# zama-ai/bounty-matrix-inversion

Measured on AMD Instinct MI355X. Metric: PBS/sec per GPU + encrypted n x n inverse wall-clock (n=2,3,4), higher is better.
Workload: dtype u64/f64

## Files before the change

bounty-matrix-inversion_amd/csrc/bmi_host.cpp:

```cpp
#include <hip/hip_runtime.h>

#include <errno.h>
#include <sys/random.h>

#include <algorithm>
#include <cmath>
#include <cstdio>
#include <cstring>
#include <string>
#include <thread>
#include <vector>

#include "../../include/bmi_tfhe.h"
#include "bmi_internal.hpp"
#include "field49.hpp"
#include "ntt_wave.hpp"
#include "ntt_half_f64.hpp"
#include "ntt_wave_f64.hpp"
#include "fft_half_f64.hpp"
#include "fft_wave_f64.hpp"
#include "fft_eighth_f64.hpp"
#include "fft_quarter_f64.hpp"
#include "t64_common.hpp"

// ... 615 lines not shown
    const int prec = c->bsk_prec;
    const hipStream_t st = c->stream;
    const char *what = "bsk_to_lat (unrolled key)";
    int rc;
    if (c->t64() && bmit::shape_supported_unrolled_fft(prec, c->P.bs_levels, c->P.bs_base_log))
        rc = build_copy(c, c->bsk3.fft_lat, bytes, what,
                        [&](double *d) { return bmit::launch_bsk_to_latf(std_polys, d, c->tw_fft_half.get(), polys, prec, st); });
    else if (c->t64())
        rc = build_copy(c, c->bsk3.exact_lat, bytes, what,
                        [&](double *d) { return bmit::launch_bsk_to_lat(std_polys, d, c->tw_half.get(), polys, prec, st); });
    else if (c->wide())
        rc = build_copy(c, c->bsk3.wide49, bytes, what,
                        [&](double *d) { return bmi49::launch_bsk_to_wide(std_polys, d, c->tw_wave.get(), c->tw_wide49.get(), polys, st); });
    else
        rc = build_copy(c, c->bsk3.lat49, bytes, what,
                        [&](double *d) { return bmi49::launch_bsk_to_lat(std_polys, d, c->tw_half.get(), polys, true, st); });
    if (rc) return rc;
    c->have_bsk3 = true;
    return 0;
}

const FieldOps GOLDILOCKS_OPS = {bmi::launch_keyswitch, bmi::launch_keyswitch_mfma, bmi::launch_ksk_to_limbs, bmi::launch_lincomb, bmi::launch_lwe_phase,
    [](bmi_ctx *c, const u64 *std_polys) { return build_copy(c, c->bsk.ntt_gl, c->bsk_std.size() * 8, "bsk_to_ntt", [&](u64 *d) {
        return bmi::launch_bsk_to_ntt(std_polys, d, c->tw_gl.get(), (uint32_t)(c->bsk_std.size() / c->N), c->stream); }); },
    [](const bmi_ctx *c, const u64 *a, const u64 *b, u64 *o, uint32_t m) { return bmi::launch_negacyclic_mul(a, b, o, c->tw_gl.get(), m, c->stream); },
    bmi::KS_LIMBS};
const FieldOps FIELD49_OPS = {bmi49::launch_keyswitch, bmi49::launch_keyswitch_mfma, bmi49::launch_ksk_to_limbs, bmi49::launch_lincomb, bmi49::launch_lwe_phase,
    [](bmi_ctx *c, const u64 *std_polys) { return build_copy(c, c->bsk.ntt49, c->bsk_std.size() * 8, "bsk_to_ntt", [&](double *d) {
        return bmi49::launch_bsk_to_ntt(std_polys, d, c->tw_wave.get(), (uint32_t)(c->bsk_std.size() / c->N), c->stream); }); },
    [](const bmi_ctx *c, const u64 *a, const u64 *b, u64 *o, uint32_t m) { return bmi49::launch_negacyclic_mul(a, b, o, c->tw_wave.get(), m, c->stream); },
    bmi49::KS_LIMBS};
const FieldOps TORUS64_OPS = {bmit::launch_keyswitch, bmit::launch_keyswitch_mfma, bmit::launch_ksk_to_limbs, bmit::launch_lincomb, bmit::launch_lwe_phase,
                              nullptr, nullptr, bmit::KS_LIMBS};

int gen_eval_keys(bmi_ctx *c, uint64_t seed) {
    HIP_OK(c, hipSetDevice(c->device));
    drop_sk_mask(c);
    const bmi_params &P = c->P;
    const uint32_t n = P.n, N = c->N, k = P.k, lk = P.ks_levels, rows = c->rows;
    c->seed = seed;
    if (!c->secure_rng) c->enc_counter = 0;
    c->bsk_std.assign((size_t)n * rows * (k + 1) * N, 0);
    gen_ggsw_rows(c, seed, S_BSK_MASK, S_BSK_NOISE, c->sk_small, c->bsk_std.data());
    c->have_bsk3 = false;
    if (c->unroll == 2) gen_bsk3(c, seed);
    c->ksk.assign((size_t)k * N * lk * (n + 1), 0);
    {
        const Stream sm_det(seed, S_KSK_MASK, c->f), se_det(seed, S_KSK_NOISE, c->f);
        const Stream *smp = &sm_det, *sep = &se_det;
        const ChaKey *ksec = &c->rng_secret, *kpub = &c->rng_public;
        const bool secure = c->secure_rng;
        const Fq f = c->f;
        const u64 *skb = c->sk_big.data();
        const u64 *sks = c->sk_small.data();
        u64 *ksk = c->ksk.data();
        const double sigma = P.lwe_noise;
        const uint32_t bl = P.ks_base_log;
        parallel_for((size_t)k * N * lk, [=](size_t jr) {
            RowRng sm(smp, *kpub, S_KSK_MASK, jr, secure), se(sep, *ksec, S_KSK_NOISE, jr, secure);
            const uint32_t j = (uint32_t)(jr / lk), lev = (uint32_t)(jr % lk);
            u64 *row = ksk + jr * (n + 1);
            u64 b = se.gauss(jr, sigma);
            for (uint32_t x = 0; x < n; x++) {
                row[x] = sm.uniform((u64)jr * (n + 1) + x);
                if (sks[x]) b = f.add(b, row[x]);
            }
            if (skb[j]) b = f.add(b, (u64)1 << (f.bits - bl * (lev + 1)));
            row[n] = b;
        });
    }
    c->have_secret = true;
    if (int rc = upload_eval_keys(c)) return rc;
    return c->unroll == 2 ? upload_bsk3(c) : 0;
}

uint32_t ks_mfma_slices(const bmi_ctx *c, uint32_t count) {
    const uint32_t tiles = (count + 31) / 32, cbs = (c->P.n + 1 + 31) / 32;
    const uint32_t ksteps = c->big_n * c->P.ks_levels / 32;
    uint32_t slices = 1;
    while (slices < 64 && slices * 2 <= ksteps && ksteps % (slices * 2) == 0 && (size_t)tiles * cbs * slices < 2048) slices *= 2;
    return slices;
}

int ensure_ks_mfma(bmi_ctx *c, uint32_t count) {
    const uint32_t cbs = (c->P.n + 1 + 31) / 32;
    const size_t sums = (size_t)ks_mfma_slices(c, count) * count * c->ops->ks_limbs * cbs * 32 * sizeof(int);
    const int rc = grow(c, c->ks_digits, (size_t)count * c->big_n * c->P.ks_levels, (size_t)8 << 20);
    return rc ? rc : grow(c, c->ks_sums, sums, (size_t)32 << 20);
}

enum class Rot {
    t64_wide2, t64_wide, t64_quad, t64_tp2u_fft, t64_lat2u_fft, t64_lat2u, t64_lat_fft, t64_lat, t64_fft, t64_exact,
    f49_wide_u, f49_wide, f49_quad, f49_lat2u, f49_lat2, f49_tpx,
    gl_lat, gl_tp,
};

int choose_rotation(const bmi_ctx *c, uint32_t count, Rot *rot) {
    if (c->unroll == 2 && !c->have_bsk3)
        return fail(c, -1, "unrolling selected but the context holds no unrolled key: generate keys after bmi_set_bsk_unroll, or bmi_import_bsk_unrolled");
    const int v = c->variant;
    const bool latency = v == 2 || (v == 0 && count <= c->lat_threshold);
    const bool two_per_wg = v == 1 || v == 3 || (v == 0 && count > 256);
    const int prec = c->bsk_prec;
    const uint32_t lv = c->P.bs_levels, bl = c->P.bs_base_log;
    if (c->t64()) {
        if (c->wide() && !c->bsk.wide2.empty() && two_per_wg) *rot = Rot::t64_wide2;
        else if (c->wide()) *rot = Rot::t64_wide;
        else if (c->quad()) *rot = Rot::t64_quad;
        else if (c->unroll == 2)
            *rot = !bmit::shape_supported_unrolled_fft(prec, lv, bl) ? Rot::t64_lat2u : two_per_wg ? Rot::t64_tp2u_fft : Rot::t64_lat2u_fft;
        else {
            if (c->bsk.fft.empty() && !bmit::shape_supported(prec, lv, bl))
                return fail(c, -1, "this bootstrap-key precision exists for the unrolled kernel only: bmi_set_bsk_unroll(ctx, 2) before keygen");
            if ((v == 5 || v == 6) && c->bsk.fft.empty())
                return fail(c, -1, "kernel variant " + std::to_string(v) + " needs the bootstrap key at 48 bits of precision in base 2^10 (the torus default)");
            const bool lat_t = v == 2 || v == 4 || v == 6 || (v == 0 && count <= c->lat_threshold);
            const bool fft = !c->bsk.fft.empty() && (lat_t ? v != 4 : v == 0 || v == 5);
            *rot = lat_t ? (fft ? Rot::t64_lat_fft : Rot::t64_lat) : (fft ? Rot::t64_fft : Rot::t64_exact);
        }
    } else if (c->f64()) {
        if (c->wide()) *rot = c->unroll == 2 ? Rot::f49_wide_u : Rot::f49_wide;
        else if (c->quad()) *rot = Rot::f49_quad;
        else *rot = c->unroll == 2 ? Rot::f49_lat2u : latency ? Rot::f49_lat2 : Rot::f49_tpx;
    } else {
        *rot = latency ? Rot::gl_lat : Rot::gl_tp;
    }
    return 0;
}

int launch_rotation(const bmi_ctx *c, Rot rot, const u64 *cts, const uint32_t *ids, uint32_t count, u64 *out, unsigned long long *stat,
                    hipStream_t st) {
    const uint32_t n = c->P.n, lv = c->P.bs_levels, bl = c->P.bs_base_log;
    const int p = c->bsk_prec;
    const u64 *luts = c->luts.get();
    const double *luts49 = reinterpret_cast<const double *>(luts);
    const bmi_ctx::BskCopies &K = c->bsk;
    const bmi_ctx::Bsk3Copies &K3 = c->bsk3;
    switch (rot) {
    case Rot::t64_wide2: return bmit::launch_blind_rotate_wide2(cts, ids, luts, K.wide2.get(), c->tw_quarter.get(), out, count, n, p, lv, bl, st);
    case Rot::t64_wide: return bmit::launch_blind_rotate_wide(cts, ids, luts, K.wide.get(), c->tw_quarter.get(), out, count, n, p, lv, bl, stat, st);
    case Rot::t64_quad: return bmit::launch_blind_rotate_quad(cts, ids, luts, K.quad.get(), c->tw_eighth.get(), out, count, n, p, lv, bl, stat, st);
    case Rot::t64_tp2u_fft: return bmit::launch_blind_rotate_tp2u_fft(cts, ids, luts, K3.fft_lat.get(), c->tw_fft_half.get(), c->zeta_pow.get(), out,
                                                                      count, n, p, lv, bl, st);
    case Rot::t64_lat2u_fft: return bmit::launch_blind_rotate_lat2u_fft(cts, ids, luts, K3.fft_lat.get(), c->tw_fft_half.get(), c->zeta_pow.get(),
                                                                        out, count, n, p, lv, bl, stat, st);
    case Rot::t64_lat2u: return bmit::launch_blind_rotate_lat2u(cts, ids, luts, K3.exact_lat.get(), c->tw_half.get(), c->root_pow.get(), out, count,
                                                                n, p, lv, bl, st);
    case Rot::t64_lat_fft: return bmit::launch_blind_rotate_lat_fft(cts, ids, luts, K.fft_lat.get(), c->tw_fft_half.get(), out, count, n, p, lv, bl, stat, st);
    case Rot::t64_lat: return bmit::launch_blind_rotate_lat(cts, ids, luts, K.exact_lat.get(), c->tw_half.get(), out, count, n, p, lv, bl, st);
    case Rot::t64_fft: return bmit::launch_blind_rotate_fft(cts, ids, luts, K.fft.get(), c->tw_fft.get(), out, count, n, p, lv, bl, stat, st);
    case Rot::t64_exact: return bmit::launch_blind_rotate(cts, ids, luts, K.exact.get(), c->tw_wave.get(), out, count, n, p, lv, bl, st);
    case Rot::f49_wide_u: return bmi49::launch_blind_rotate_wide_u(cts, ids, luts49, K3.wide49.get(), c->tw_wave.get(), c->tw_wide49.get(),
                                                                   c->root_pow.get(), out, count, n, lv, bl, st);
    case Rot::f49_wide: return bmi49::launch_blind_rotate_wide(cts, ids, luts49, K.wide49.get(), c->tw_wave.get(), c->tw_wide49.get(), out, count, n, lv, bl, st);
    case Rot::f49_quad: return bmi49::launch_blind_rotate_quad(cts, ids, luts49, K.quad49.get(), c->tw_wave.get(), c->tw_quad49.get(), out, count, n, st);
    case Rot::f49_lat2u: return bmi49::launch_blind_rotate_lat2u(cts, ids, luts49, K3.lat49.get(), c->tw_half.get(), c->root_pow.get(), out, count, n, lv, bl, st);
    case Rot::f49_lat2: return bmi49::launch_blind_rotate_lat2(cts, ids, luts49, K.lat49.get(), c->tw_half.get(), out, count, n, lv, bl, st);
    case Rot::f49_tpx: return bmi49::launch_blind_rotate_tpx(cts, ids, luts49, K.ntt49.get(), c->tw_wave.get(), out, count, n, lv, bl, st);
    case Rot::gl_lat: return bmi::launch_blind_rotate_lat(cts, ids, luts, K.ntt_gl.get(), c->tw_gl.get(), out, count, n, st);
    case Rot::gl_tp: return bmi::launch_blind_rotate_tp(cts, ids, luts, K.ntt_gl.get(), c->tw_gl.get(), out, count, n, st);
    }
    return (int)hipErrorInvalidValue;
}

int check_lut_ids(bmi_ctx *c, const uint32_t *lut_ids, uint32_t count) {
    for (uint32_t i = 0; i < count; i++)
        if (lut_ids[i] >= c->n_luts) return fail(c, -1, "look-up id " + std::to_string(lut_ids[i]) + " is not registered");
    return 0;
}

}
// ... 440 lines not shown
        while (slices < 64 && tiles * slices * 2 <= 1024) slices *= 2;
    if (slices > 1)
        if (int rc = grow(c, c->ks_partial, (size_t)slices * count * c->ks_stride * 16, KS_PARTIAL_BYTES)) return rc;
    int rc = c->ops->keyswitch(d_in, c->ksk_padded.get(), c->ks_bias.get(), d_small, slices > 1 ? c->ks_partial.get() : nullptr, slices,
                               count, c->P.n, c->big_n, c->P.ks_levels, c->P.ks_base_log, c->ks_stride, (hipStream_t)stream);
    return rc ? fail(c, -2, std::string("keyswitch launch: ") + hipGetErrorString((hipError_t)rc)) : 0;
}

int bmi_blind_rotate_batch(bmi_ctx *c, const uint64_t *d_small, const uint32_t *d_lut_ids, uint32_t count,
                           uint64_t *d_out, void *stream) {
    if (!c || (count && (!d_small || !d_lut_ids || !d_out))) return -1;
    if (!c->have_keys) return fail(c, -1, "no keys: call bmi_keygen first");
    HIP_OK(c, hipSetDevice(c->device));
    Rot rot;
    if (int rc = choose_rotation(c, count, &rot)) return rc;
    if (rot == Rot::t64_lat || rot == Rot::t64_exact)
        if (int rc = build_exact_torus_copies(c, nullptr)) return rc;
    const int rc = launch_rotation(c, rot, d_small, d_lut_ids, count, d_out, nullptr, (hipStream_t)stream);
    return rc ? fail(c, -2, std::string("blind_rotate launch: ") + hipGetErrorString((hipError_t)rc)) : 0;
}

int bmi_pbs_batch(bmi_ctx *c, const uint64_t *d_in, const uint32_t *d_lut_ids, uint32_t count, uint64_t *d_out,
                  void *stream) {
    if (!c) return -1;
    HIP_OK(c, hipSetDevice(c->device));
    int rc = ensure_small(c, count);
    if (rc) return rc;
    rc = bmi_keyswitch_batch(c, d_in, count, c->small.get(), stream);
    if (rc) return rc;
    return bmi_blind_rotate_batch(c, c->small.get(), d_lut_ids, count, d_out, stream);
}

int bmi_lincomb_batch(bmi_ctx *c, const uint64_t *d_store, const uint32_t *d_row_ptr, const uint32_t *d_idx,
                      const int64_t *d_coef, const uint64_t *d_const_body, uint32_t count, uint64_t *d_out,
                      void *stream) {
    if (!c || (count && (!d_store || !d_row_ptr || !d_const_body || !d_out))) return -1;
    HIP_OK(c, hipSetDevice(c->device));
    int rc = c->ops->lincomb(d_store, d_row_ptr, d_idx, (const i64 *)d_coef, d_const_body, d_out, count, c->big_n + 1, (hipStream_t)stream);
    return rc ? fail(c, -2, std::string("lincomb launch: ") + hipGetErrorString((hipError_t)rc)) : 0;
}

static int phase_decrypt_batch(bmi_ctx *c, const uint64_t *d_ct, uint32_t count, uint32_t delta_log, const int64_t *d_expected,
                               uint64_t *d_phase, int64_t *d_msgs, int64_t *d_err, void *stream) {
    if (!c->have_keys) return fail(c, -1, "no keys: call bmi_keygen first");
    if (!c->have_secret) return fail(c, -1, "evaluation-only context: it holds no secret key");
    if (count == 0) return 0;
    HIP_OK(c, hipSetDevice(c->device));
    if (int rc = ensure_sk_mask(c)) return rc;
    const int rc = c->ops->lwe_phase(d_ct, c->sk_mask.get(), d_phase, (const i64 *)d_expected, (i64 *)d_msgs, (i64 *)d_err, count, c->big_n,
                                     delta_log, (hipStream_t)stream);
    return rc ? fail(c, -2, std::string("lwe_phase launch: ") + hipGetErrorString((hipError_t)rc)) : 0;
}

int bmi_phase_batch(bmi_ctx *c, const uint64_t *d_ct, uint32_t count, uint64_t *d_phase, void *stream) {
    if (!c || (count && (!d_ct || !d_phase))) return -1;
    return phase_decrypt_batch(c, d_ct, count, 0, nullptr, d_phase, nullptr, nullptr, stream);
}

int bmi_decrypt_batch(bmi_ctx *c, const uint64_t *d_ct, uint32_t count, uint32_t delta_log, const int64_t *d_expected,
                      int64_t *d_msgs, int64_t *d_err, void *stream) {
    if (!c || (count && (!d_ct || !d_msgs))) return -1;
    if (delta_log == 0 || delta_log >= c->f.bits - 1) return fail(c, -1, "delta_log out of range");
    return phase_decrypt_batch(c, d_ct, count, delta_log, d_expected, nullptr, d_msgs, d_err, stream);
}

int bmi_scatter_rows(bmi_ctx *c, const uint64_t *d_src, uint32_t count, uint64_t *d_store, const uint32_t *d_rows,
                     void *stream) {
    if (!c || (count && (!d_src || !d_store || !d_rows))) return -1;
    HIP_OK(c, hipSetDevice(c->device));
    int rc = bmi::launch_scatter_rows(d_src, d_store, d_rows, count, c->big_n + 1, (hipStream_t)stream);
    return rc ? fail(c, -2, std::string("scatter_rows launch: ") + hipGetErrorString((hipError_t)rc)) : 0;
}

int bmi_reserve(bmi_ctx *c, uint32_t max_count) {
    if (!c) return -1;
    HIP_OK(c, hipSetDevice(c->device));
    HIP_OK(c, hipDeviceSynchronize());
    if (int rc = grow(c, c->ks_partial, KS_PARTIAL_BYTES, KS_PARTIAL_BYTES)) return rc;
    if (c->ks_mfma_ok) {
        uint32_t worst = max_count;
        size_t worst_sums = 0;
        for (uint32_t tiles = 1; tiles <= (max_count + 31) / 32; tiles++) {
            const uint32_t cnt = std::min(tiles * 32, max_count);
            const size_t sums = (size_t)ks_mfma_slices(c, cnt) * cnt;
            if (sums > worst_sums) { worst_sums = sums; worst = cnt; }
        }
        int rc = ensure_ks_mfma(c, worst);
        if (rc) return rc;
        rc = ensure_ks_mfma(c, max_count);
        if (rc) return rc;
    }
    return ensure_small(c, max_count);
}

int bmi_sync(bmi_ctx *c, void *stream) {
    if (!c) return -1;
    HIP_OK(c, hipStreamSynchronize((hipStream_t)stream));
    return 0;
}

int bmi_pbs_batch_host(bmi_ctx *c, const uint64_t *in, const uint32_t *lut_ids, uint32_t count, uint64_t *out) {
    if (!c || !in || !lut_ids || !out) return -1;
    if (int bad = check_lut_ids(c, lut_ids, count)) return bad;
    HIP_OK(c, hipSetDevice(c->device));
    int rc = ensure_io(c, count);
    if (rc) return rc;
    const size_t w = (size_t)(c->big_n + 1) * 8;
    HIP_OK(c, hipMemcpyAsync(c->io_a.get(), in, count * w, hipMemcpyHostToDevice, c->stream));
    HIP_OK(c, hipMemcpyAsync(c->io_ids.get(), lut_ids, count * 4, hipMemcpyHostToDevice, c->stream));
    rc = bmi_pbs_batch(c, c->io_a.get(), c->io_ids.get(), count, c->io_b.get(), c->stream);
    if (rc) return rc;
    HIP_OK(c, hipMemcpyAsync(out, c->io_b.get(), count * w, hipMemcpyDeviceToHost, c->stream));
    HIP_OK(c, hipStreamSynchronize(c->stream));
    return 0;
}

int bmi_keyswitch_batch_host(bmi_ctx *c, const uint64_t *in, uint32_t count, uint64_t *small_out) {
    if (!c || !in || !small_out) return -1;
    HIP_OK(c, hipSetDevice(c->device));
    int rc = ensure_io(c, count);
    if (rc) return rc;
    HIP_OK(c, hipMemcpyAsync(c->io_a.get(), in, (size_t)count * (c->big_n + 1) * 8, hipMemcpyHostToDevice, c->stream));
    rc = bmi_keyswitch_batch(c, c->io_a.get(), count, c->small.get(), c->stream);
    if (rc) return rc;
    HIP_OK(c, hipMemcpyAsync(small_out, c->small.get(), (size_t)count * (c->P.n + 1) * 8, hipMemcpyDeviceToHost, c->stream));
    HIP_OK(c, hipStreamSynchronize(c->stream));
    return 0;
}

int bmi_blind_rotate_batch_host(bmi_ctx *c, const uint64_t *small_in, const uint32_t *lut_ids, uint32_t count,
                                uint64_t *out) {
    if (!c || !small_in || !lut_ids || !out) return -1;
    if (int bad = check_lut_ids(c, lut_ids, count)) return bad;
    HIP_OK(c, hipSetDevice(c->device));
    int rc = ensure_io(c, count);
    if (rc) return rc;
    HIP_OK(c, hipMemcpyAsync(c->small.get(), small_in, (size_t)count * (c->P.n + 1) * 8, hipMemcpyHostToDevice, c->stream));
    HIP_OK(c, hipMemcpyAsync(c->io_ids.get(), lut_ids, count * 4, hipMemcpyHostToDevice, c->stream));
    rc = bmi_blind_rotate_batch(c, c->small.get(), c->io_ids.get(), count, c->io_b.get(), c->stream);
    if (rc) return rc;
    HIP_OK(c, hipMemcpyAsync(out, c->io_b.get(), (size_t)count * (c->big_n + 1) * 8, hipMemcpyDeviceToHost, c->stream));
    HIP_OK(c, hipStreamSynchronize(c->stream));
    return 0;
}

int bmi_fft_margin_host(bmi_ctx *c, const uint64_t *small_in, const uint32_t *lut_ids, uint32_t count, uint64_t *out,
                        double *max_distance) {
    if (!c || !small_in || !lut_ids || !out || !max_distance) return -1;
    if (!c->have_keys) return fail(c, -1, "no keys: call bmi_keygen first");
    const bool ufft = c->t64() && c->unroll == 2 && c->have_bsk3 && bmit::shape_supported_unrolled_fft(c->bsk_prec, c->P.bs_levels, c->P.bs_base_log);
    const bool wide_key = !c->bsk.wide.empty() || !c->bsk.quad.empty();
    if (c->bsk.fft.empty() && !wide_key && !ufft)
        return fail(c, -1, "the floating-point-transform kernels exist on the 2^64 torus with the bootstrap key at 48 bits (N = 1024), 46 bits "
                           "(N = 2048) or 44 bits (N = 4096) in base 2^10");
    const Rot rot = ufft ? Rot::t64_lat2u_fft : !wide_key && (c->variant == 6 || c->variant == 2) ? Rot::t64_lat_fft
                    : wide_key ? (c->quad() ? Rot::t64_quad : Rot::t64_wide) : Rot::t64_fft;
    if (int bad = check_lut_ids(c, lut_ids, count)) return bad;
    HIP_OK(c, hipSetDevice(c->device));
    int rc = ensure_io(c, count);
    if (rc) return rc;
    DevBuf<unsigned long long> d_stat;
    HIP_OK(c, d_stat.alloc(8));
    hipError_t e = hipMemsetAsync(d_stat.get(), 0, 8, c->stream);
    if (e == hipSuccess) e = hipMemcpyAsync(c->small.get(), small_in, (size_t)count * (c->P.n + 1) * 8, hipMemcpyHostToDevice, c->stream);
    if (e == hipSuccess) e = hipMemcpyAsync(c->io_ids.get(), lut_ids, count * 4, hipMemcpyHostToDevice, c->stream);
    if (e == hipSuccess) e = (hipError_t)launch_rotation(c, rot, c->small.get(), c->io_ids.get(), count, c->io_b.get(), d_stat.get(), c->stream);
    unsigned long long bits = 0;
// ... 26 lines not shown
```

bounty-matrix-inversion_amd/csrc/bmi_internal.hpp:

```cpp
#pragma once
#include <hip/hip_runtime.h>
#include <stdint.h>

#include "goldilocks.hpp"

#ifndef BMI_DEFAULT_Q_BITS
#define BMI_DEFAULT_Q_BITS 65
#endif

#ifndef BMI_TPX49_PF
#define BMI_TPX49_PF 13
#endif

#ifndef BMI_TPX49_RESYNC
#define BMI_TPX49_RESYNC 4
#endif

#define BMI_LUT_CAP 1024
#define BMI_MAX_LWE_N 1024
constexpr int BMI_AT_WORDS = 264;
constexpr int BMI_LDS_WORDS_MAX = 160 * 1024 / 8;
#ifndef BMI_KS_MFMA_MIN
#define BMI_KS_MFMA_MIN 1
#endif
// ... 33 lines not shown
    BMI_LAUNCH_CHECK();
    return 0;
}

template <typename F>
inline int with_levels(uint32_t levels, F f) {
    if (levels == 3) return f(std::integral_constant<int, 3>{});
    return f(std::integral_constant<int, 2>{});
}
template <typename F>
inline int with_levels_stats(uint32_t levels, bool stats, F f) {
    return with_levels(levels, [&](auto L) { return stats ? f(L, std::true_type{}) : f(L, std::false_type{}); });
}

namespace bmi {
using gl::i64;
using gl::u64;

int launch_bsk_to_ntt(const u64 *std_polys, u64 *ntt_polys, const u64 *g_tw, uint32_t n_polys, hipStream_t s);
int launch_negacyclic_mul(const u64 *a, const u64 *b, u64 *c, const u64 *g_tw, uint32_t count, hipStream_t s);
int launch_blind_rotate_tp(const u64 *small_cts, const uint32_t *lut_ids, const u64 *luts, const u64 *bsk,
                           const u64 *g_tw, u64 *out, uint32_t count, uint32_t n, hipStream_t s);
int launch_blind_rotate_lat(const u64 *small_cts, const uint32_t *lut_ids, const u64 *luts, const u64 *bsk,
                            const u64 *g_tw, u64 *out, uint32_t count, uint32_t n, hipStream_t s);
int launch_keyswitch(const u64 *in, const u64 *ksk, const u64 *ks_bias, u64 *out, void *partial, uint32_t slices,
                     uint32_t count, uint32_t n, uint32_t big_n, uint32_t levels, uint32_t base_log, uint32_t ks_stride,
                     hipStream_t s);
constexpr uint32_t KS_LIMBS = 9;
int launch_ksk_to_limbs(const u64 *ksk, signed char *limbs, uint32_t rows, uint32_t n, uint32_t ks_stride, hipStream_t s);
int launch_keyswitch_mfma(const u64 *in, const signed char *limbs, signed char *digits, int *sums, u64 *out,
                          uint32_t slices, uint32_t count, uint32_t n, uint32_t big_n, uint32_t levels,
                          uint32_t base_log, hipStream_t s);
int launch_lincomb(const u64 *store, const uint32_t *row_ptr, const uint32_t *idx, const i64 *coef,
                   const u64 *const_body, u64 *out, uint32_t count, uint32_t width, hipStream_t s);
int launch_scatter_rows(const u64 *src, u64 *store, const uint32_t *rows, uint32_t count, uint32_t width, hipStream_t s);
int launch_lwe_phase(const u64 *ct, const u64 *key_mask, u64 *phase, const i64 *expected, i64 *msgs, i64 *err,
                     uint32_t count, uint32_t big_n, uint32_t delta_log, hipStream_t s);
}

namespace bmi49 {
using gl::i64;
using gl::u64;
int launch_bsk_to_ntt(const u64 *std_polys, double *ntt_polys, const double *g_tw, uint32_t n_polys, hipStream_t s);
int launch_negacyclic_mul(const u64 *a, const u64 *b, u64 *c, const double *g_tw, uint32_t count, hipStream_t s);
int launch_bsk_to_quad(const u64 *std_polys, double *quad_polys, const double *g_tw, const double *g_t, uint32_t n_polys,
                       hipStream_t s);
int launch_blind_rotate_quad(const u64 *small_cts, const uint32_t *lut_ids, const double *luts, const double *bsk_quad,
                             const double *g_tw, const double *g_t, u64 *out, uint32_t count, uint32_t n, hipStream_t s);
int launch_bsk_to_wide(const u64 *std_polys, double *wide_polys, const double *g_tw, const double *g_tw_wide,
                       uint32_t n_polys, hipStream_t s);
int launch_blind_rotate_wide(const u64 *small_cts, const uint32_t *lut_ids, const double *luts, const double *bsk_wide,
                             const double *g_tw, const double *g_tw_wide, u64 *out, uint32_t count, uint32_t n,
                             uint32_t levels, uint32_t base_log, hipStream_t s);
int launch_blind_rotate_wide_u(const u64 *small_cts, const uint32_t *lut_ids, const double *luts, const double *bsk3_wide,
                               const double *g_tw, const double *g_tw_wide, const double *g_root_pow, u64 *out, uint32_t count,
                               uint32_t n, uint32_t levels, uint32_t base_log, hipStream_t s);
int launch_bsk_to_lat(const u64 *std_polys, double *lat_polys, const double *g_tw_h, uint32_t n_polys, bool paired, hipStream_t s);
int launch_blind_rotate_lat2(const u64 *small_cts, const uint32_t *lut_ids, const double *luts, const double *bsk_lat,
                             const double *g_tw_h, u64 *out, uint32_t count, uint32_t n, uint32_t levels, uint32_t base_log,
                             hipStream_t s);
int launch_blind_rotate_lat2u(const u64 *small_cts, const uint32_t *lut_ids, const double *luts, const double *bsk3_lat,
                              const double *g_tw_h, const double *g_root_pow, u64 *out, uint32_t count, uint32_t n,
                              uint32_t levels, uint32_t base_log, hipStream_t s);
int launch_blind_rotate_tpx(const u64 *small_cts, const uint32_t *lut_ids, const double *luts, const double *bsk,
                            const double *g_tw, u64 *out, uint32_t count, uint32_t n, uint32_t levels, uint32_t base_log,
                            hipStream_t s);
int launch_keyswitch(const u64 *in, const u64 *ksk, const u64 *ks_bias, u64 *out, void *partial, uint32_t slices,
                     uint32_t count, uint32_t n, uint32_t big_n, uint32_t levels, uint32_t base_log, uint32_t ks_stride,
                     hipStream_t s);
constexpr uint32_t KS_LIMBS = 7;
int launch_ksk_to_limbs(const u64 *ksk, signed char *limbs, uint32_t rows, uint32_t n, uint32_t ks_stride, hipStream_t s);
int launch_keyswitch_mfma(const u64 *in, const signed char *limbs, signed char *digits, int *sums, u64 *out,
                          uint32_t slices, uint32_t count, uint32_t n, uint32_t big_n, uint32_t levels,
                          uint32_t base_log, hipStream_t s);
int launch_lincomb(const u64 *store, const uint32_t *row_ptr, const uint32_t *idx, const i64 *coef,
                   const u64 *const_body, u64 *out, uint32_t count, uint32_t width, hipStream_t s);
int launch_lwe_phase(const u64 *ct, const u64 *key_mask, u64 *phase, const i64 *expected, i64 *msgs, i64 *err,
                     uint32_t count, uint32_t big_n, uint32_t delta_log, hipStream_t s);
}

namespace bmit {
using gl::i64;
using gl::u64;
constexpr uint32_t KS_LIMBS = 9;
bool shape_supported(int prec, uint32_t levels, uint32_t base_log);
bool shape_supported_unrolled(int prec, uint32_t levels, uint32_t base_log);
int launch_bsk_to_limbs(const u64 *std_polys, double *limb_polys, const double *g_tw, uint32_t n_polys, int prec,
                        hipStream_t s);
int launch_blind_rotate(const u64 *small_cts, const uint32_t *lut_ids, const u64 *luts, const double *bsk_limbs,
                        const double *g_tw, u64 *out, uint32_t count, uint32_t n, int prec, uint32_t levels,
                        uint32_t base_log, hipStream_t s);
int launch_bsk_to_lat(const u64 *std_polys, double *lat_polys, const double *g_tw_h, uint32_t n_polys, int prec, hipStream_t s);
int launch_blind_rotate_lat(const u64 *small_cts, const uint32_t *lut_ids, const u64 *luts, const double *bsk_lat,
                            const double *g_tw_h, u64 *out, uint32_t count, uint32_t n, int prec, uint32_t levels,
                            uint32_t base_log, hipStream_t s);
int launch_blind_rotate_lat2u(const u64 *small_cts, const uint32_t *lut_ids, const u64 *luts, const double *bsk3_lat,
                              const double *g_tw_h, const double *g_root_pow, u64 *out, uint32_t count, uint32_t n, int prec,
                              uint32_t levels, uint32_t base_log, hipStream_t s);
bool shape_supported_fft(int prec, uint32_t levels, uint32_t base_log);
int launch_bsk_to_fft(const u64 *std_polys, double *limb_polys, const double *g_tw_fft, uint32_t n_polys, int prec, hipStream_t s);
int launch_blind_rotate_fft(const u64 *small_cts, const uint32_t *lut_ids, const u64 *luts, const double *bsk_fft,
                            const double *g_tw_fft, u64 *out, uint32_t count, uint32_t n, int prec, uint32_t levels,
                            uint32_t base_log, unsigned long long *stat, hipStream_t s);
int launch_bsk_to_latf(const u64 *std_polys, double *lat_polys, const double *g_tw_h, uint32_t n_polys, int prec, hipStream_t s);
int launch_blind_rotate_lat_fft(const u64 *small_cts, const uint32_t *lut_ids, const u64 *luts, const double *bsk_fft,
                                const double *g_tw_fft, u64 *out, uint32_t count, uint32_t n, int prec, uint32_t levels,
                                uint32_t base_log, unsigned long long *stat, hipStream_t s);
bool shape_supported_unrolled_fft(int prec, uint32_t levels, uint32_t base_log);
int launch_blind_rotate_lat2u_fft(const u64 *small_cts, const uint32_t *lut_ids, const u64 *luts, const double *bsk3_latf,
                                  const double *g_tw_h, const double *g_zeta_pow, u64 *out, uint32_t count, uint32_t n, int prec,
                                  uint32_t levels, uint32_t base_log, unsigned long long *stat, hipStream_t s);
int launch_blind_rotate_tp2u_fft(const u64 *small_cts, const uint32_t *lut_ids, const u64 *luts, const double *bsk3_latf,
                                 const double *g_tw_h, const double *g_zeta_pow, u64 *out, uint32_t count, uint32_t n, int prec,
                                 uint32_t levels, uint32_t base_log, hipStream_t s);
bool shape_supported_quad(int prec, uint32_t levels, uint32_t base_log);
int launch_bsk_to_quad(const u64 *std_polys, double *q_polys, const double *g_tw_e, uint32_t n_polys, int prec, hipStream_t s);
int launch_blind_rotate_quad(const u64 *small_cts, const uint32_t *lut_ids, const u64 *luts, const double *bsk_q, const double *g_tw_e,
                             u64 *out, uint32_t count, uint32_t n, int prec, uint32_t levels, uint32_t base_log, unsigned long long *stat,
                             hipStream_t s);
int launch_bsk_to_wide2(const u64 *std_polys, double *w2_polys, const double *g_tw_q, uint32_t n_polys, int prec, hipStream_t s);
int launch_blind_rotate_wide2(const u64 *small_cts, const uint32_t *lut_ids, const u64 *luts, const double *bsk_w2, const double *g_tw_q,
                              u64 *out, uint32_t count, uint32_t n, int prec, uint32_t levels, uint32_t base_log, hipStream_t s);
bool shape_supported_wide(int prec, uint32_t levels, uint32_t base_log);
int launch_bsk_to_wide(const u64 *std_polys, double *w_polys, const double *g_tw_q, uint32_t n_polys, int prec, hipStream_t s);
int launch_blind_rotate_wide(const u64 *small_cts, const uint32_t *lut_ids, const u64 *luts, const double *bsk_w, const double *g_tw_q,
                             u64 *out, uint32_t count, uint32_t n, int prec, uint32_t levels, uint32_t base_log, unsigned long long *stat,
                             hipStream_t s);
int launch_keyswitch(const u64 *in, const u64 *ksk, const u64 *ks_bias, u64 *out, void *partial, uint32_t slices,
                     uint32_t count, uint32_t n, uint32_t big_n, uint32_t levels, uint32_t base_log, uint32_t ks_stride,
                     hipStream_t s);
int launch_ksk_to_limbs(const u64 *ksk, signed char *limbs, uint32_t rows, uint32_t n, uint32_t ks_stride, hipStream_t s);
int launch_keyswitch_mfma(const u64 *in, const signed char *limbs, signed char *digits, int *sums, u64 *out,
                          uint32_t slices, uint32_t count, uint32_t n, uint32_t big_n, uint32_t levels,
                          uint32_t base_log, hipStream_t s);
int launch_lincomb(const u64 *store, const uint32_t *row_ptr, const uint32_t *idx, const i64 *coef,
                   const u64 *const_body, u64 *out, uint32_t count, uint32_t width, hipStream_t s);
int launch_lwe_phase(const u64 *ct, const u64 *key_mask, u64 *phase, const i64 *expected, i64 *msgs, i64 *err,
                     uint32_t count, uint32_t big_n, uint32_t delta_log, hipStream_t s);
}
```

bounty-matrix-inversion_amd/csrc/ks_mfma.hpp:

```cpp
#pragma once
#include <hip/hip_runtime.h>
#include <stdint.h>

#include "bmi_internal.hpp"

namespace ksm {

typedef uint64_t u64;
typedef int64_t i64;
typedef int v4i __attribute__((ext_vector_type(4)));
typedef int v16i __attribute__((ext_vector_type(16)));

constexpr int TILE = 32;
constexpr int KSTEP = 32;
constexpr int WAVES = 4;
#ifndef BMI_KS_PF_WIDE
#define BMI_KS_PF_WIDE 3
#endif
#ifndef BMI_KS_PF
#define BMI_KS_PF 4
#endif

template <class F>
__global__ void __launch_bounds__(256)
    k_ks_digits(const u64 *__restrict__ in, signed char *__restrict__ D, uint32_t count, uint32_t big_n, uint32_t levels,
                uint32_t base_log) {
    const size_t idx = (size_t)blockIdx.x * blockDim.x + threadIdx.x;
    if (idx >= (size_t)count * big_n) return;
    const uint32_t ct = (uint32_t)(idx / big_n), j = (uint32_t)(idx % big_n);
    unsigned char d[16];
    F::digits(in[(size_t)ct * (big_n + 1) + j], levels, base_log, d);
    const int half = 1 << (base_log - 1);
    signed char *o = D + ((size_t)ct * big_n + j) * levels;
    if ((levels & 7) == 0) {
        for (uint32_t g = 0; g < levels; g += 8) {
            u64 w = 0;
#pragma unroll
            for (int lev = 0; lev < 8; lev++) w |= (u64)(unsigned char)(signed char)((int)d[g + lev] - half) << (8 * lev);
            *reinterpret_cast<u64 *>(o + g) = w;
        }
    } else {
        for (uint32_t lev = 0; lev < levels; lev++) o[lev] = (signed char)((int)d[lev] - half);
    }
}

__host__ __device__ __forceinline__ size_t limb_offset(uint32_t cb, uint32_t ks, uint32_t limb, uint32_t h, uint32_t r,
                                                       uint32_t ksteps, uint32_t L) {
    return (((((size_t)cb * ksteps + ks) * L + limb) * 2 + h) * 32 + r) * 16;
}

template <class F>
__global__ void __launch_bounds__(256)
    k_ksk_to_limbs(const u64 *__restrict__ ksk, signed char *__restrict__ Bm, uint32_t rows, uint32_t n, uint32_t ks_stride,
                   uint32_t L) {
    const uint32_t cbs = (n + 1 + TILE - 1) / TILE, ksteps = rows / KSTEP;
    const size_t idx = (size_t)blockIdx.x * blockDim.x + threadIdx.x;
    if (idx >= (size_t)rows * cbs * TILE) return;
    const uint32_t col = (uint32_t)(idx % (cbs * TILE)), k = (uint32_t)(idx / (cbs * TILE));
    __int128 c = col <= n ? (__int128)F::centered(ksk[(size_t)k * ks_stride + col]) : 0;
    const uint32_t cb = col / TILE, r = col % TILE, ks = k / KSTEP, h = (k % KSTEP) / 16, byte = k % 16;
    for (uint32_t l = 0; l < L; l++) {
        const int dl = (int)((c + 128) & 255) - 128;
        c = (c - dl) >> 8;
        Bm[limb_offset(cb, ks, l, h, r, ksteps, L) + byte] = (signed char)dl;
    }
}

template <int L>
constexpr int ks_pf() { return L <= 7 ? BMI_KS_PF : BMI_KS_PF_WIDE; }

template <int L>
__global__ void __launch_bounds__(64 * WAVES)
    k_ks_mfma(const signed char *__restrict__ D, const signed char *__restrict__ Bm, int *__restrict__ S, uint32_t count,
              uint32_t K, uint32_t cbs, uint32_t ksteps_per_slice) {
    const int wave = threadIdx.x >> 6, lane = threadIdx.x & 63;
    const uint32_t tile = blockIdx.x * WAVES + wave;
    if (tile * TILE >= count) return;
    const uint32_t cb = blockIdx.y, slice = blockIdx.z;
    const uint32_t r = lane & 31, h = lane >> 5;
    const uint32_t ksteps = K / KSTEP;
    const uint32_t ks0 = slice * ksteps_per_slice;
    const uint32_t ks1 = min(ks0 + ksteps_per_slice, ksteps);
    const uint32_t ct_row = min(tile * TILE + r, count - 1);
    const v4i *ap = reinterpret_cast<const v4i *>(D + (size_t)ct_row * K + 16 * h) + (size_t)ks0 * 2;
    const v4i *bp = reinterpret_cast<const v4i *>(Bm + limb_offset(cb, ks0, 0, h, r, ksteps, L));
    constexpr int BSTEP = L * 64;

    v16i acc[L];
#pragma unroll
    for (int l = 0; l < L; l++)
#pragma unroll
        for (int i = 0; i < 16; i++) acc[l][i] = 0;

    constexpr int KS_PF = ks_pf<L>();
    v4i a_buf[KS_PF], b_buf[KS_PF][L];
#pragma unroll
    for (int s = 0; s < KS_PF; s++) {
        a_buf[s] = v4i{0, 0, 0, 0};
#pragma unroll
        for (int l = 0; l < L; l++) b_buf[s][l] = v4i{0, 0, 0, 0};
        if (ks0 + s < ks1) {
            a_buf[s] = ap[2 * s];
#pragma unroll
            for (int l = 0; l < L; l++) b_buf[s][l] = bp[s * BSTEP + l * 64];
        }
    }
    for (uint32_t ks = ks0; ks < ks1; ks += KS_PF) {
#pragma unroll
        for (int s = 0; s < KS_PF; s++) {
            if (ks + s < ks1) {
#pragma unroll
                for (int l = 0; l < L; l++) acc[l] = __builtin_amdgcn_mfma_i32_32x32x32_i8(a_buf[s], b_buf[s][l], acc[l], 0, 0, 0);
                if (ks + s + KS_PF < ks1) {
                    a_buf[s] = ap[2 * (s + KS_PF)];
#pragma unroll
                    for (int l = 0; l < L; l++) b_buf[s][l] = bp[(s + KS_PF) * BSTEP + l * 64];
                }
            }
        }
        ap += 2 * KS_PF;
        bp += (size_t)BSTEP * KS_PF;
    }

    const uint32_t cw = cbs * TILE;
#pragma unroll
    for (int i = 0; i < 16; i++) {
        const uint32_t row = (i & 3) + 8 * (i >> 2) + 4 * h;
        const uint32_t ct = tile * TILE + row;
        if (ct >= count) continue;
        int *o = S + (((size_t)slice * count + ct) * L) * cw + cb * TILE + r;
#pragma unroll
        for (int l = 0; l < L; l++) o[(size_t)l * cw] = acc[l][i];
    }
}

template <class F, int L>
__global__ void __launch_bounds__(256)
    k_ks_combine(const u64 *__restrict__ in, const int *__restrict__ S, u64 *__restrict__ out, uint32_t count, uint32_t n,
                 uint32_t big_n, uint32_t cbs, uint32_t slices) {
    const uint32_t ct = blockIdx.x;
    const uint32_t cw = cbs * TILE;
    for (uint32_t col = threadIdx.x; col <= n; col += blockDim.x) {
        i64 sum[L];
#pragma unroll
        for (int l = 0; l < L; l++) sum[l] = 0;
#pragma unroll 4
        for (uint32_t sl = 0; sl < slices; sl++) {
            const int *base = S + (((size_t)sl * count + ct) * L) * cw + col;
#pragma unroll
            for (int l = 0; l < L; l++) sum[l] += base[(size_t)l * cw];
        }
        __int128 v = 0;
#pragma unroll
        for (int l = L - 1; l >= 0; l--) v = v * 256 + sum[l];
        const bool neg = v < 0;
        const unsigned __int128 m = neg ? (unsigned __int128)(-v) : (unsigned __int128)v;
        u64 red = F::reduce128((u64)(m >> 64), (u64)m);
        if (neg) red = F::neg(red);
        const u64 base = col == n ? in[(size_t)ct * (big_n + 1) + big_n] : 0;
        out[(size_t)ct * (n + 1) + col] = F::sub(base, red);
    }
}

inline size_t limb_bytes(uint32_t rows, uint32_t n, uint32_t L) {
    const uint32_t cbs = (n + 1 + TILE - 1) / TILE;
    return (size_t)cbs * (rows / KSTEP) * L * 2 * 32 * 16;
}
inline size_t s_bytes(uint32_t count, uint32_t n, uint32_t L, uint32_t slices) {
    const uint32_t cbs = (n + 1 + TILE - 1) / TILE;
    return (size_t)slices * count * L * cbs * TILE * sizeof(int);
}

template <class F>
int launch_ksk_to_limbs(const u64 *ksk, signed char *Bm, uint32_t rows, uint32_t n, uint32_t ks_stride, uint32_t L,
                        hipStream_t s) {
    const uint32_t cbs = (n + 1 + TILE - 1) / TILE;
    const size_t total = (size_t)rows * cbs * TILE;
    hipLaunchKernelGGL((k_ksk_to_limbs<F>), dim3((unsigned)((total + 255) / 256)), dim3(256), 0, s, ksk, Bm, rows, n,
                       ks_stride, L);
    BMI_LAUNCH_CHECK();
    return 0;
}

template <class F, int L>
int launch_keyswitch(const u64 *in, const signed char *Bm, signed char *D, int *S, u64 *out, uint32_t slices,
                     uint32_t count, uint32_t n, uint32_t big_n, uint32_t levels, uint32_t base_log, hipStream_t s) {
    if (count == 0) return 0;
    const uint32_t K = big_n * levels, cbs = (n + 1 + TILE - 1) / TILE, ksteps = K / KSTEP;
    const size_t coefs = (size_t)count * big_n;
    hipLaunchKernelGGL((k_ks_digits<F>), dim3((unsigned)((coefs + 255) / 256)), dim3(256), 0, s, in, D, count, big_n, levels,
                       base_log);
    BMI_LAUNCH_CHECK();
    const uint32_t tiles = (count + TILE - 1) / TILE;
    const uint32_t per_slice = (ksteps + slices - 1) / slices;
    hipLaunchKernelGGL((k_ks_mfma<L>), dim3((tiles + WAVES - 1) / WAVES, cbs, slices), dim3(64 * WAVES), 0, s, D, Bm, S, count,
                       K, cbs, per_slice);
    BMI_LAUNCH_CHECK();
    hipLaunchKernelGGL((k_ks_combine<F, L>), dim3(count), dim3(256), 0, s, in, S, out, count, n, big_n, cbs, slices);
    BMI_LAUNCH_CHECK();
    return 0;
}

}
```

Measured before the change: 121,100.

## Stage keyswitch MFMA B-tiles through LDS and fuse combine when unsliced

The int8 MFMA keyswitch kernel now loads the key-limb tiles cooperatively into a double-buffered shared-memory stage, with register prefetch, instead of each wave loading its own copy from global memory. When only one K-slice is used, recombination and reduction are fused into the MFMA epilogue, which skips the partial-sum buffer and the separate combine launch. The T64 keyswitch limb count drops from 9 to 8, reducing MFMA and memory work per step, and sum-buffer sizing skips allocation when unsliced. In exchange it adds per-step barriers and LDS traffic, and the limb change relies on 8 limbs still covering the needed precision.

```diff
diff --git a/bounty-matrix-inversion_amd/csrc/bmi_host.cpp b/bounty-matrix-inversion_amd/csrc/bmi_host.cpp
--- a/bounty-matrix-inversion_amd/csrc/bmi_host.cpp
+++ b/bounty-matrix-inversion_amd/csrc/bmi_host.cpp
@@ -721,11 +721,16 @@
     return slices;
 }
 
+size_t ks_sum_words(const bmi_ctx *c, uint32_t count) {
+    const uint32_t slices = ks_mfma_slices(c, count);
+    return slices > 1 ? (size_t)slices * count : 0;
+}
+
 int ensure_ks_mfma(bmi_ctx *c, uint32_t count) {
     const uint32_t cbs = (c->P.n + 1 + 31) / 32;
-    const size_t sums = (size_t)ks_mfma_slices(c, count) * count * c->ops->ks_limbs * cbs * 32 * sizeof(int);
+    const size_t sums = ks_sum_words(c, count) * c->ops->ks_limbs * cbs * 32 * sizeof(int);
     const int rc = grow(c, c->ks_digits, (size_t)count * c->big_n * c->P.ks_levels, (size_t)8 << 20);
-    return rc ? rc : grow(c, c->ks_sums, sums, (size_t)32 << 20);
+    return rc || !sums ? rc : grow(c, c->ks_sums, sums, (size_t)32 << 20);
 }
 
 enum class Rot {
@@ -1332,7 +1337,7 @@
         size_t worst_sums = 0;
         for (uint32_t tiles = 1; tiles <= (max_count + 31) / 32; tiles++) {
             const uint32_t cnt = std::min(tiles * 32, max_count);
-            const size_t sums = (size_t)ks_mfma_slices(c, cnt) * cnt;
+            const size_t sums = ks_sum_words(c, cnt);
             if (sums > worst_sums) { worst_sums = sums; worst = cnt; }
         }
         int rc = ensure_ks_mfma(c, worst);
diff --git a/bounty-matrix-inversion_amd/csrc/bmi_internal.hpp b/bounty-matrix-inversion_amd/csrc/bmi_internal.hpp
--- a/bounty-matrix-inversion_amd/csrc/bmi_internal.hpp
+++ b/bounty-matrix-inversion_amd/csrc/bmi_internal.hpp
@@ -139,7 +139,7 @@
 namespace bmit {
 using gl::i64;
 using gl::u64;
-constexpr uint32_t KS_LIMBS = 9;
+constexpr uint32_t KS_LIMBS = 8;
 bool shape_supported(int prec, uint32_t levels, uint32_t base_log);
 bool shape_supported_unrolled(int prec, uint32_t levels, uint32_t base_log);
 int launch_bsk_to_limbs(const u64 *std_polys, double *limb_polys, const double *g_tw, uint32_t n_polys, int prec,
diff --git a/bounty-matrix-inversion_amd/csrc/ks_mfma.hpp b/bounty-matrix-inversion_amd/csrc/ks_mfma.hpp
--- a/bounty-matrix-inversion_amd/csrc/ks_mfma.hpp
+++ b/bounty-matrix-inversion_amd/csrc/ks_mfma.hpp
@@ -1,6 +1,8 @@
 #pragma once
 #include <hip/hip_runtime.h>
 #include <stdint.h>
+
+#include <type_traits>
 
 #include "bmi_internal.hpp"
 
@@ -66,25 +68,41 @@
     }
 }
 
+template <class F, int L>
+__device__ __forceinline__ u64 ks_recombine(const i64 (&sum)[L], u64 base) {
+    __int128 v = 0;
+#pragma unroll
+    for (int l = L - 1; l >= 0; l--) v = v * 256 + sum[l];
+    const bool neg = v < 0;
+    const unsigned __int128 m = neg ? (unsigned __int128)(-v) : (unsigned __int128)v;
+    u64 red = F::reduce128((u64)(m >> 64), (u64)m);
+    if (neg) red = F::neg(red);
+    return F::sub(base, red);
+}
+
 template <int L>
-constexpr int ks_pf() { return L <= 7 ? BMI_KS_PF : BMI_KS_PF_WIDE; }
-
-template <int L>
+constexpr int ks_pf() { return L <= 8 ? BMI_KS_PF : BMI_KS_PF_WIDE; }
+
+template <class F, int L, bool FUSED>
 __global__ void __launch_bounds__(64 * WAVES)
-    k_ks_mfma(const signed char *__restrict__ D, const signed char *__restrict__ Bm, int *__restrict__ S, uint32_t count,
-              uint32_t K, uint32_t cbs, uint32_t ksteps_per_slice) {
+    k_ks_mfma(const signed char *__restrict__ D, const signed char *__restrict__ Bm, int *__restrict__ S,
+              const u64 *__restrict__ in, u64 *__restrict__ out, uint32_t count, uint32_t K, uint32_t cbs,
+              uint32_t ksteps_per_slice, uint32_t n, uint32_t big_n) {
     const int wave = threadIdx.x >> 6, lane = threadIdx.x & 63;
     const uint32_t tile = blockIdx.x * WAVES + wave;
-    if (tile * TILE >= count) return;
     const uint32_t cb = blockIdx.y, slice = blockIdx.z;
     const uint32_t r = lane & 31, h = lane >> 5;
     const uint32_t ksteps = K / KSTEP;
     const uint32_t ks0 = slice * ksteps_per_slice;
     const uint32_t ks1 = min(ks0 + ksteps_per_slice, ksteps);
+    const uint32_t nsteps = ks1 > ks0 ? ks1 - ks0 : 0;
     const uint32_t ct_row = min(tile * TILE + r, count - 1);
     const v4i *ap = reinterpret_cast<const v4i *>(D + (size_t)ct_row * K + 16 * h) + (size_t)ks0 * 2;
-    const v4i *bp = reinterpret_cast<const v4i *>(Bm + limb_offset(cb, ks0, 0, h, r, ksteps, L));
     constexpr int BSTEP = L * 64;
+    constexpr int THREADS = 64 * WAVES;
+    constexpr int NW = (BSTEP + THREADS - 1) / THREADS;
+    const v4i *bg = reinterpret_cast<const v4i *>(Bm + limb_offset(cb, ks0, 0, 0, 0, ksteps, L));
+    __shared__ v4i stage[2][BSTEP];
 
     v16i acc[L];
 #pragma unroll
@@ -93,33 +111,56 @@
         for (int i = 0; i < 16; i++) acc[l][i] = 0;
 
     constexpr int KS_PF = ks_pf<L>();
-    v4i a_buf[KS_PF], b_buf[KS_PF][L];
-#pragma unroll
-    for (int s = 0; s < KS_PF; s++) {
-        a_buf[s] = v4i{0, 0, 0, 0};
-#pragma unroll
-        for (int l = 0; l < L; l++) b_buf[s][l] = v4i{0, 0, 0, 0};
-        if (ks0 + s < ks1) {
-            a_buf[s] = ap[2 * s];
-#pragma unroll
-            for (int l = 0; l < L; l++) b_buf[s][l] = bp[s * BSTEP + l * 64];
-        }
-    }
-    for (uint32_t ks = ks0; ks < ks1; ks += KS_PF) {
+    constexpr int UNROLL = KS_PF % 2 ? 2 * KS_PF : KS_PF;
+    v4i a_buf[KS_PF], g_buf[KS_PF][NW], b_reg[2][L];
+
+    if (nsteps) {
+        const uint32_t last = nsteps - 1;
+        const auto a_at = [&](uint32_t step) __attribute__((always_inline)) { return ap[2 * (size_t)min(step, last)]; };
+        const auto b_at = [&](uint32_t step, int j) __attribute__((always_inline)) {
+            const uint32_t w = j * THREADS + threadIdx.x;
+            return bg[(size_t)min(step, last) * BSTEP + ((j + 1) * THREADS <= BSTEP ? w : min(w, (uint32_t)BSTEP - 1))];
+        };
+        const auto b_put = [&](int st, int j, v4i v) __attribute__((always_inline)) {
+            if ((j + 1) * THREADS <= BSTEP || j * THREADS + threadIdx.x < BSTEP) stage[st][j * THREADS + threadIdx.x] = v;
+        };
+#pragma unroll
+        for (int st = 0; st < 2; st++)
+#pragma unroll
+            for (int j = 0; j < NW; j++) b_put(st, j, b_at(st, j));
 #pragma unroll
         for (int s = 0; s < KS_PF; s++) {
-            if (ks + s < ks1) {
-#pragma unroll
-                for (int l = 0; l < L; l++) acc[l] = __builtin_amdgcn_mfma_i32_32x32x32_i8(a_buf[s], b_buf[s][l], acc[l], 0, 0, 0);
-                if (ks + s + KS_PF < ks1) {
-                    a_buf[s] = ap[2 * (s + KS_PF)];
-#pragma unroll
-                    for (int l = 0; l < L; l++) b_buf[s][l] = bp[(s + KS_PF) * BSTEP + l * 64];
+            a_buf[s] = a_at(s);
+#pragma unroll
+            for (int j = 0; j < NW; j++) g_buf[s][j] = b_at(s + 2, j);
+        }
+        __syncthreads();
+#pragma unroll
+        for (int l = 0; l < L; l++) b_reg[0][l] = stage[0][l * 64 + lane];
+
+        const auto trip = [&](uint32_t i, auto guarded) __attribute__((always_inline)) {
+#pragma unroll
+            for (int u = 0; u < UNROLL; u++) {
+                constexpr bool G = decltype(guarded)::value;
+                const int s = u % KS_PF;
+                if (!G || i + u < nsteps) {
+                    __syncthreads();
+#pragma unroll
+                    for (int l = 0; l < L; l++) {
+                        acc[l] = __builtin_amdgcn_mfma_i32_32x32x32_i8(a_buf[s], b_reg[u & 1][l], acc[l], 0, 0, 0);
+                        b_reg[(u + 1) & 1][l] = stage[(u + 1) & 1][l * 64 + lane];
+                        if (l >= L - NW) b_put(u & 1, l - (L - NW), g_buf[s][l - (L - NW)]);
+                        __builtin_amdgcn_sched_barrier(0);
+                    }
+#pragma unroll
+                    for (int j = 0; j < NW; j++) g_buf[s][j] = b_at(i + u + 2 + KS_PF, j);
+                    a_buf[s] = a_at(i + u + KS_PF);
                 }
             }
-        }
-        ap += 2 * KS_PF;
-        bp += (size_t)BSTEP * KS_PF;
+        };
+        uint32_t i = 0;
+        for (; i + UNROLL <= nsteps; i += UNROLL) trip(i, std::false_type{});
+        if (i < nsteps) trip(i, std::true_type{});
     }
 
     const uint32_t cw = cbs * TILE;
@@ -128,9 +169,19 @@
         const uint32_t row = (i & 3) + 8 * (i >> 2) + 4 * h;
         const uint32_t ct = tile * TILE + row;
         if (ct >= count) continue;
-        int *o = S + (((size_t)slice * count + ct) * L) * cw + cb * TILE + r;
-#pragma unroll
-        for (int l = 0; l < L; l++) o[(size_t)l * cw] = acc[l][i];
+        if constexpr (FUSED) {
+            const uint32_t col = cb * TILE + r;
+            if (col > n) continue;
+            i64 sum[L];
+#pragma unroll
+            for (int l = 0; l < L; l++) sum[l] = acc[l][i];
+            const u64 base = col == n ? in[(size_t)ct * (big_n + 1) + big_n] : 0;
+            out[(size_t)ct * (n + 1) + col] = ks_recombine<F, L>(sum, base);
+        } else {
+            int *o = S + (((size_t)slice * count + ct) * L) * cw + cb * TILE + r;
+#pragma unroll
+            for (int l = 0; l < L; l++) o[(size_t)l * cw] = acc[l][i];
+        }
     }
 }
 
@@ -150,15 +201,8 @@
 #pragma unroll
             for (int l = 0; l < L; l++) sum[l] += base[(size_t)l * cw];
         }
-        __int128 v = 0;
-#pragma unroll
-        for (int l = L - 1; l >= 0; l--) v = v * 256 + sum[l];
-        const bool neg = v < 0;
-        const unsigned __int128 m = neg ? (unsigned __int128)(-v) : (unsigned __int128)v;
-        u64 red = F::reduce128((u64)(m >> 64), (u64)m);
-        if (neg) red = F::neg(red);
         const u64 base = col == n ? in[(size_t)ct * (big_n + 1) + big_n] : 0;
-        out[(size_t)ct * (n + 1) + col] = F::sub(base, red);
+        out[(size_t)ct * (n + 1) + col] = ks_recombine<F, L>(sum, base);
     }
 }
 
@@ -193,8 +237,13 @@
     BMI_LAUNCH_CHECK();
     const uint32_t tiles = (count + TILE - 1) / TILE;
     const uint32_t per_slice = (ksteps + slices - 1) / slices;
-    hipLaunchKernelGGL((k_ks_mfma<L>), dim3((tiles + WAVES - 1) / WAVES, cbs, slices), dim3(64 * WAVES), 0, s, D, Bm, S, count,
-                       K, cbs, per_slice);
+    const dim3 grid((tiles + WAVES - 1) / WAVES, cbs, slices);
+    if (slices == 1) {
+        hipLaunchKernelGGL((k_ks_mfma<F, L, true>), grid, dim3(64 * WAVES), 0, s, D, Bm, S, in, out, count, K, cbs, per_slice, n, big_n);
+        BMI_LAUNCH_CHECK();
+        return 0;
+    }
+    hipLaunchKernelGGL((k_ks_mfma<F, L, false>), grid, dim3(64 * WAVES), 0, s, D, Bm, S, in, out, count, K, cbs, per_slice, n, big_n);
     BMI_LAUNCH_CHECK();
     hipLaunchKernelGGL((k_ks_combine<F, L>), dim3(count), dim3(256), 0, s, in, S, out, count, n, big_n, cbs, slices);
     BMI_LAUNCH_CHECK();
```

Result: no change. 121,800, median of 6 (+0.6%).
